# nem0/LumixEngine

Hardware: AMD Instinct MI355X
Metric: entities_culled_per_sec (higher is better)
Workload: dtype f32; 1 GPU; BASELINE config 2: 10000000 static entities per GPU (sparse, cube +-15000), 1 frustum (fov 60, 16:9, near 0.1, far 10000), cull + compaction; entities_per_gpu=10000000, frusta=1, repetitions=1

## Files before the change

lumixengine_amd/csrc/cull_kernels.hip:

```cpp
#include <algorithm>
#include <cstddef>
#include <cstdlib>

#include "lmx_kernels.h"
#include <type_traits>

#include <hip/hip_ext.h>

namespace lmx {

namespace {

__device__ __forceinline__ uint32_t lane_id() { return __builtin_amdgcn_mbcnt_hi(~0u, __builtin_amdgcn_mbcnt_lo(~0u, 0u)); }
__device__ __forceinline__ uint32_t mbcnt64(uint64_t mask) {
	return __builtin_amdgcn_mbcnt_hi((uint32_t)(mask >> 32), __builtin_amdgcn_mbcnt_lo((uint32_t)mask, 0u));
}
typedef uint32_t u32x4_a4 __attribute__((ext_vector_type(4), aligned(4)));
__device__ __forceinline__ float readlane_f(float v, int lane) { return __uint_as_float(__builtin_amdgcn_readlane(__float_as_uint(v), lane)); }

struct TileScalars {
	uint32_t ent_begin, cell_cap, n_frusta;
	uint32_t keys_packed;
	uint32_t out_stride, cnt_pad, cnt_frustum_stride, n_zero;
	int32_t* out_slots;
// ... 65 lines not shown
	const double cs = (double)CELL_SIZE;
	const double ox = org[0], oy = org[1], oz = org[2];
	const float lx = (float)(cs * bi[0] - cs - ox), ly = (float)(cs * bi[1] - cs - oy), lz = (float)(cs * bi[2] - cs - oz);
	const float hx = (float)(cs * bi[3] + cs - ox), hy = (float)(cs * bi[4] + cs - oy), hz = (float)(cs * bi[5] + cs - oz);
	const float clx = (float)(cs * bi[0] + cs - ox), cly = (float)(cs * bi[1] + cs - oy), clz = (float)(cs * bi[2] + cs - oz);
	const float chx = (float)(cs * bi[3] + 2 * cs - ox), chy = (float)(cs * bi[4] + 2 * cs - oy), chz = (float)(cs * bi[5] + 2 * cs - oz);
	const float b1 = max_f(abs_f(lx), abs_f(chx)) + max_f(abs_f(ly), abs_f(chy)) + max_f(abs_f(lz), abs_f(chz));
	const float n1 = abs_f(nx) + abs_f(ny) + abs_f(nz);
	const float margin = max_f(1.0f, n1) * (2.0f + 4e-6f * b1) + 1e-6f * abs_f(d);
	bool rej, in;
	{
		const float bx = nx > 0.0f ? hx : lx, by = ny > 0.0f ? hy : ly, bz = nz > 0.0f ? hz : lz;
		const float dp = (nx * bx) + (ny * by) + (nz * bz);
		rej = dp < -d - margin;
	}
	{
		const float bx = nx < 0.0f ? chx : clx, by = ny < 0.0f ? chy : cly, bz = nz < 0.0f ? chz : clz;
		const float dp = (nx * bx) + (ny * by) + (nz * bz);
		in = dp > -d + margin;
	}
	const uint64_t rej_mask = __ballot(plane_lane && rej), out_mask = __ballot(plane_lane && !in);
	uint32_t st_bits = 0;
	for (int g = 0; g < nf; ++g) {
		const uint32_t r = (uint32_t)(rej_mask >> (6 * g)) & 63u, o = (uint32_t)(out_mask >> (6 * g)) & 63u;
		st_bits |= (r != 0 ? (uint32_t)TILE_REJECT : (o == 0 ? (uint32_t)TILE_ACCEPT : (uint32_t)TILE_MIXED)) << (2 * g);
	}
	return st_bits;
}


typedef float v2f __attribute__((ext_vector_type(2)));
typedef float f32x16 __attribute__((ext_vector_type(16)));
typedef float v4f_t __attribute__((ext_vector_type(4)));
typedef uint32_t u32x4_t __attribute__((ext_vector_type(4)));
typedef __bf16 bf16x2_t __attribute__((ext_vector_type(2)));
typedef __bf16 bf16x8_t __attribute__((ext_vector_type(8)));
__device__ __forceinline__ uint32_t pk_bf16(float a, float b) { const v2f v = {a, b}; return __builtin_bit_cast(uint32_t, __builtin_convertvector(v, bf16x2_t)); }
typedef float v8f_t __attribute__((ext_vector_type(8)));
__device__ __forceinline__ float min3_drop_nan(float a, float b, float c) { return fminf(fminf(a, b), c); }
__device__ __forceinline__ bool sphere_visible_d_pk(const DevFrustum& f, const float d[6], float cx, float cy, float cz, float radius) {
	const v2f x2 = {cx, cx}, y2 = {cy, cy}, z2 = {cz, cz}, r2 = {radius, radius};
	bool culled = false;
#pragma unroll
	for (int k = 0; k < 6; k += 2) {
		const v2f nx = {f.nx[k], f.nx[k + 1]}, ny = {f.ny[k], f.ny[k + 1]}, nz = {f.nz[k], f.nz[k + 1]}, dd = {d[k], d[k + 1]};
		v2f t = x2 * nx;
		t = t + y2 * ny;
		t = t + z2 * nz;
		t = t + dd;
		t = t + r2;
		culled = culled || (t.x < 0) || (t.y < 0);
	}
	return !culled;
}


struct alignas(16) CellInfo { float d[6]; uint32_t cls, pad; };
static_assert(sizeof(CellInfo) == 32, "two ds_read_b128 per (lane, chunk, frustum)");

#ifndef LMX_ASM_SGPR
#define LMX_ASM_SGPR(x) "+s"(x)
#endif
#define LMX_CULL_WAVES_ATTR(F) __attribute__((amdgpu_waves_per_eu((F) == 1 ? 1 : 5)))

template <int F, int WAVES, int CHW, int GRP, int FORM, int SLOTS_I>
__global__ __launch_bounds__(WAVES * 64) LMX_CULL_WAVES_ATTR(F) void k_cull_tile(const FrustaArg fr_arg, const float4* __restrict__ g_spheres, const int32_t* __restrict__ g_ids,
	const ChunkHdr* __restrict__ g_hdr, const CellKey* __restrict__ g_tile_cells, const uint32_t* __restrict__ g_tile_tab, const TileBox* __restrict__ g_tile_box,
	const uint2* __restrict__ g_tile_out, int32_t* __restrict__ g_out_ids, uint32_t* __restrict__ g_counts, uint32_t* __restrict__ g_counts_next, const TileScalars a) {
	constexpr bool SLOTS = SLOTS_I != 0;
	constexpr uint32_t TILE = WAVES * CHW * 64;
	constexpr uint32_t THREADS = WAVES * 64;
	constexpr int FS = F == 1 ? 1 : MAX_FRUSTA;
	static_assert(CHW * FS <= 32, "visibility bits of a wave's chunks x frusta live in one register");
	LMX_DYNAMIC_LDS(CellInfo, s_info);
	__shared__ __attribute__((aligned(16))) float s_nrm[F != 1 ? MAX_FRUSTA : 1][F != 1 ? 20 : 4];
	const DevFrustum* __restrict__ frp = (const DevFrustum*)__builtin_amdgcn_kernarg_segment_ptr();
	const int nf = F == 1 ? 1 : (int)a.n_frusta;

	const uint32_t lane = lane_id();
	const uint32_t wave = __builtin_amdgcn_readfirstlane(threadIdx.x >> 6);
	const uint32_t tile_ent = a.ent_begin + blockIdx.x * TILE;
	const uint32_t tile_index = tile_ent / TILE;

	for (uint32_t i = blockIdx.x * THREADS + threadIdx.x; i < a.n_zero; i += gridDim.x * THREADS) g_counts_next[i] = 0;

	uint32_t st_bits = 0, tile_flags = 0, plane_skip = 0;
	bool any_mixed = false, any_live = false;
	if constexpr (FORM != 0) {
		static_assert(F == 1, "the lane-parallel tile test handles one frustum");
		__shared__ uint32_t s_verdict;
		if (wave == 0) {
			const uint32_t v = tile_status_lanes(g_tile_box + tile_index, lane);
			if (lane == 0) s_verdict = v;
		}
		__syncthreads();
		const uint32_t r = s_verdict;
		st_bits = r & 3u;
		tile_flags = (r >> 2) & 63u;
		plane_skip = __builtin_amdgcn_readfirstlane((r >> 8) & 63u);
		any_mixed = st_bits == TILE_MIXED;
		any_live = st_bits != TILE_REJECT;
	} else {
		__shared__ uint32_t s_verdict_multi[2];
		if (wave == 0) {
			uint32_t fl;
			const uint32_t v = tile_status_lanes_multi(g_tile_box + tile_index, lane, nf, &fl);
			if (lane == 0) {
				s_verdict_multi[0] = v;
				s_verdict_multi[1] = fl;
			}
		}
		__syncthreads();
		st_bits = __builtin_amdgcn_readfirstlane(s_verdict_multi[0]);
		tile_flags = __builtin_amdgcn_readfirstlane(s_verdict_multi[1]);
		static_assert(TILE_REJECT == 0 && TILE_ACCEPT == 1 && TILE_MIXED == 2, "the verdicts of all frusta are read off the 2-bit fields by bit logic");
		any_mixed = ((st_bits >> 1) & ~st_bits & 0x5555u) != 0;
		any_live = st_bits != 0;
	}
	if (!any_live) return;
	uint32_t tile_word = 0;
	v2f* s_d2 = reinterpret_cast<v2f*>(s_info);
	uint32_t* s_word = reinterpret_cast<uint32_t*>(s_d2 + (F != 1 ? (size_t)nf * a.cell_cap * 3 : 0));
	constexpr bool SPLIT = F != 1 && WAVES == 4;
	uint16_t* s_w16 = reinterpret_cast<uint16_t*>(s_word);
	if constexpr (F != 1) {
		static_assert(TILE_ACCEPT == 1 && CELL_ACCEPT == 1, "a settled frustum contributes CELL_ACCEPT or nothing: its verdict field IS its class field");
		tile_word = st_bits & ~(st_bits >> 1) & 0x5555u;
	}

	constexpr bool STREAMING = F == 1 && (FORM == 2 || FORM == 4);
	constexpr bool PRELOAD = STREAMING || F != 1;
	typedef float v4f_pre __attribute__((ext_vector_type(4)));
	v4f_pre pre_sp[PRELOAD ? GRP : 1];
	int32_t pre_id[PRELOAD ? GRP : 1];
	auto preload_group0 = [&](auto with_spheres) {
		if constexpr (PRELOAD) {
			const size_t e0 = ((size_t)((tile_ent >> 6) + wave * CHW) << 6) + lane;
#pragma unroll
			for (int i = 0; i < GRP; ++i) {
				pre_id[i] = __builtin_nontemporal_load(g_ids + e0 + i * 64);
				if constexpr (decltype(with_spheres)::value) pre_sp[i] = __builtin_nontemporal_load(reinterpret_cast<const v4f_pre*>(g_spheres + e0 + i * 64));
			}
		}
	};
	uint32_t first_cell = 0;
	if (any_mixed) {
		first_cell = g_tile_tab[2 * tile_index];
		const uint32_t n_cells = g_tile_tab[2 * tile_index + 1];
		const bool packed_keys = F == 1 ? FORM <= 2 : a.keys_packed != 0;
		const char* keys = reinterpret_cast<const char*>(g_tile_cells) + ((size_t)tile_index * a.cell_cap << (packed_keys ? 3 : 4));
		struct FetchedKey { uint4 raw; int32_t lo[3]; };
		auto fetch_key = [&](uint32_t t) -> FetchedKey {
			FetchedKey k;
			if (packed_keys) {
				const uint2 raw = reinterpret_cast<const uint2*>(keys)[t];
				k.raw = uint4{raw.x, raw.y, 0u, 0u};
				uint32_t zero = 0;
				asm volatile("" : "+v"(zero));
				const int32_t* box_lo = reinterpret_cast<const int32_t*>(g_tile_box + tile_index) + zero;
				k.lo[0] = box_lo[0]; k.lo[1] = box_lo[1]; k.lo[2] = box_lo[2];
			} else {
				k.raw = reinterpret_cast<const uint4*>(keys)[t];
				k.lo[0] = k.lo[1] = k.lo[2] = 0;
			}
			return k;
		};
		auto decode_key = [&](const FetchedKey& k) -> CellKey {
// ... 550 lines not shown

__global__ __launch_bounds__(256) void k_apply_patches(float4* __restrict__ spheres, int32_t* __restrict__ ids, TileBox* __restrict__ box0,
	TileBox* __restrict__ box1, TileBox* __restrict__ box2, DynDeviceView d, const PatchSphere* __restrict__ ps, uint32_t n_ps,
	const PatchId* __restrict__ pi, uint32_t n_pi, const PatchDyn* __restrict__ pd, uint32_t n_pd) {
	uint32_t i = blockIdx.x * 256u + threadIdx.x;
	if (i < n_ps) {
		const PatchSphere p = ps[i];
		spheres[p.slot] = make_float4(p.x, p.y, p.z, p.radius);
		return;
	}
	i -= n_ps;
	if (i < n_pi) {
		const PatchId p = pi[i];
		ids[p.slot] = p.id;
		if (p.id < 0) {
			atomicAnd(&box0[p.slot >> 12].flags, ~(uint32_t)TILE_DENSE);
			atomicAnd(&box1[p.slot >> 11].flags, ~(uint32_t)TILE_DENSE);
			atomicAnd(&box2[p.slot >> 10].flags, ~(uint32_t)TILE_DENSE);
		}
		return;
	}
	i -= n_pi;
	if (i < n_pd) {
		const PatchDyn p = pd[i];
		d.px[p.slot] = p.px;
		d.py[p.slot] = p.py;
		d.pz[p.slot] = p.pz;
		d.radius[p.slot] = p.radius;
		d.ids[p.slot] = p.id;
	}
}

constexpr int FIN_THREADS = 256;
constexpr int FIN_MAX_SHARDS = 1024;
__global__ __launch_bounds__(FIN_THREADS) void k_cull_finalize(const uint32_t* __restrict__ counts, uint32_t cnt_pad, uint32_t cnt_frustum_stride,
	const uint8_t* __restrict__ shard_type, uint32_t n_shards, uint32_t* __restrict__ totals, uint32_t* __restrict__ pref, uint32_t* __restrict__ packed_start) {
	__shared__ uint32_t s_cnt[FIN_MAX_SHARDS];
	__shared__ uint8_t s_type[FIN_MAX_SHARDS];
	__shared__ uint32_t s_tot[MAX_TYPES];
	const uint32_t f = blockIdx.x;
	const uint32_t t = threadIdx.x;
	if (t < MAX_TYPES) s_tot[t] = 0;
	for (uint32_t s = t; s < n_shards; s += FIN_THREADS) {
		s_cnt[s] = counts[f * cnt_frustum_stride + s * cnt_pad];
		s_type[s] = shard_type[s];
	}
	__syncthreads();
	for (uint32_t s = t; s < n_shards; s += FIN_THREADS) {
		const uint8_t ty = s_type[s];
		uint32_t run = 0;
		for (uint32_t k = s; k-- > 0 && s_type[k] == ty;) run += s_cnt[k];
		pref[f * n_shards + s] = run;
		if (s + 1 == n_shards || s_type[s + 1] != ty) s_tot[ty] = run + s_cnt[s];
	}
	__syncthreads();
	if (t < MAX_TYPES) {
		totals[f * MAX_TYPES + t] = s_tot[t];
		if (packed_start != nullptr) {
			uint32_t at = 0;
			for (uint32_t k = 0; k < t; ++k) at += s_tot[k];
			packed_start[f * MAX_TYPES + t] = at;
		}
	}
}

__global__ __launch_bounds__(256) void k_cull_consolidate(const int32_t* __restrict__ src, uint32_t src_stride, const uint32_t* __restrict__ win_base,
	const uint32_t* __restrict__ counts, uint32_t cnt_pad, uint32_t cnt_frustum_stride, const uint8_t* __restrict__ shard_type,
	const uint32_t* __restrict__ type_start, uint32_t type_start_stride, const uint32_t* __restrict__ pref, uint32_t n_shards, int32_t* __restrict__ dst,
	uint32_t dst_stride, uint32_t dst_cap, const int32_t* __restrict__ src2 ,
	int32_t* __restrict__ dst2) {
	const uint32_t s = blockIdx.x, f = blockIdx.y;
	const uint32_t c = counts[f * cnt_frustum_stride + s * cnt_pad];
	const size_t from_at = (size_t)f * src_stride + win_base[s];
	const uint32_t at = type_start[f * type_start_stride + shard_type[s]] + pref[f * n_shards + s];
	const size_t to_at = (size_t)f * dst_stride + at;
	const uint32_t room = at < dst_cap ? dst_cap - at : 0u;
	const uint32_t n = c < room ? c : room;
	for (uint32_t k = blockIdx.z * 256u + threadIdx.x; k < n; k += gridDim.z * 256u) {
		dst[to_at + k] = src[from_at + k];
		if (src2 != nullptr) dst2[to_at + k] = src2[from_at + k];
	}
}

__global__ __launch_bounds__(256) void k_cull_pack(const int32_t* __restrict__ src, const uint32_t* __restrict__ win_base, const uint32_t* __restrict__ counts,
	uint32_t cnt_pad, const uint8_t* __restrict__ shard_type, uint32_t n_shards, int32_t* __restrict__ rec_base, PackLayout lay,
	uint32_t src_stride, uint32_t cnt_stride) {
	__shared__ uint32_t s_part[4];
	__shared__ uint32_t s_tot[MAX_TYPES];
	const uint32_t s = blockIdx.x, t = threadIdx.x;
	src += (size_t)blockIdx.z * src_stride;
	counts += (size_t)blockIdx.z * cnt_stride;
	uint32_t* const header = reinterpret_cast<uint32_t*>(rec_base + lay.off[blockIdx.z]);
	int32_t* const dst = rec_base + lay.off[blockIdx.z] + MAX_TYPES;
	const uint32_t dst_cap = lay.cap[blockIdx.z];
	const bool totals_block = s == 0 && blockIdx.y == 0;
	const uint32_t c = counts[s * cnt_pad];
	if (blockIdx.y * 256u >= c && !totals_block) return;
	const int32_t* from = src + win_base[s];
	const uint32_t k0 = blockIdx.y * 256u + t;
	const int32_t first = k0 < c ? from[k0] : 0;
	uint32_t before = 0;
	for (uint32_t k = t; k < s; k += 256u) before += counts[k * cnt_pad];
#pragma unroll
	for (int o = 32; o > 0; o >>= 1) before += (uint32_t)__shfl_xor((int)before, o);
	if ((t & 63u) == 0) s_part[t >> 6] = before;
	if (totals_block && t < MAX_TYPES) s_tot[t] = 0;
	__syncthreads();
	const uint32_t at = s_part[0] + s_part[1] + s_part[2] + s_part[3];
	if (totals_block) {
		for (uint32_t k = t; k < n_shards; k += 256u) atomicAdd(&s_tot[shard_type[k]], counts[k * cnt_pad]);
		__syncthreads();
		if (t < MAX_TYPES) header[t] = s_tot[t];
	}
	int32_t* to = dst + at;
	const uint32_t room = at < dst_cap ? dst_cap - at : 0u;
	const uint32_t n = c < room ? c : room;
	if (k0 < n) to[k0] = first;
	for (uint32_t k = k0 + gridDim.y * 256u; k < n; k += gridDim.y * 256u) to[k] = from[k];
}

template <int F, int WAVES, int CHW, int GRP, int FORM, int SLOTS_I>
hipError_t tile_f(hipStream_t s, const CullDeviceView& v, uint32_t ent_begin, uint32_t ent_end, const TypeTable& tt, const FrustaArg& fr, int n_frusta,
	const CullOut& out) {
	constexpr uint32_t TILE = WAVES * CHW * 64;
	static_assert(TILE_ALIGN % TILE == 0, "tiles must not straddle type ranges");
	constexpr int K = TILE == 4096 ? 0 : (TILE == 2048 ? 1 : 2);
	const uint32_t tiles = (ent_end - ent_begin) / TILE;
	if (!tiles) {
		if (out.ev_start != nullptr) {
			(void)hipEventRecord(out.ev_start, s);
			(void)hipEventRecord(out.ev_stop, s);
		}
		return hipSuccess;
	}
	TileScalars a;
	(void)tt;
	a.ent_begin = ent_begin;
	a.cell_cap = v.tile_cap[K];
	a.keys_packed = v.keys_packed ? 1u : 0u;
	a.n_frusta = (uint32_t)n_frusta;
	a.out_stride = out.stride;
	a.cnt_pad = out.cnt_pad;
	a.cnt_frustum_stride = out.cnt_frustum_stride;
	a.n_zero = out.n_zero;
	a.out_slots = out.slots;
	{
		float n1 = 0.f;
		bool finite = true;
		for (int f = 0; f < n_frusta; ++f) {
			for (int k = 0; k < 6; ++k) {
				const float v = (__builtin_fabsf(fr.f[f].nx[k]) + __builtin_fabsf(fr.f[f].ny[k])) + __builtin_fabsf(fr.f[f].nz[k]);
				finite = finite && v <= 3.0e38f;
				n1 = v > n1 ? v : n1;
			}
		}
		a.pretest_n1s = finite ? n1 * 1.000001f * 134217728.0f : __builtin_inff();
	}
	if (out.ev_start != nullptr)
		hipExtLaunchKernelGGL((k_cull_tile<F, WAVES, CHW, GRP, FORM, SLOTS_I>), dim3(tiles), dim3(WAVES * 64), cull_tile_lds_bytes(n_frusta, a.cell_cap), s, out.ev_start, out.ev_stop, 0, fr,
			v.spheres, v.ids, v.hdr, v.tile_cells[K], v.tile_tab[K], v.tile_box[K], v.tile_out[K], out.ids, out.counts, out.counts_next, a);
	else
		hipLaunchKernelGGL((k_cull_tile<F, WAVES, CHW, GRP, FORM, SLOTS_I>), dim3(tiles), dim3(WAVES * 64), cull_tile_lds_bytes(n_frusta, a.cell_cap), s, fr, v.spheres, v.ids, v.hdr,
			v.tile_cells[K], v.tile_tab[K], v.tile_box[K], v.tile_out[K], out.ids, out.counts, out.counts_next, a);
	return hipGetLastError();
}

}

size_t cull_tile_lds_bytes(int n_frusta, uint32_t cell_cap) {
	return n_frusta > 1 ? (size_t)n_frusta * cell_cap * 24 + (size_t)cell_cap * (n_frusta > 4 ? 8 : 4) : (size_t)cell_cap * sizeof(CellInfo);
}

uint32_t cull_tile_size(int n_frusta, int variant) {
	(void)variant;
	return n_frusta <= 4 ? 2048u : 1024u;
}

hipError_t launch_cull_tile(hipStream_t s, const CullDeviceView& v, uint32_t ent_begin, uint32_t ent_end, const TypeTable& tt, const FrustaArg& fr,
	int n_frusta, const CullOut& out, int variant) {
#define LMX_TILE(F, W, C, G, L) return out.slots ? tile_f<F, W, C, G, L, 1>(s, v, ent_begin, ent_end, tt, fr, n_frusta, out) : tile_f<F, W, C, G, L, 0>(s, v, ent_begin, ent_end, tt, fr, n_frusta, out)
	if (n_frusta < 1 || n_frusta > MAX_FRUSTA) return hipErrorInvalidValue;
	if (n_frusta == 1) {
		const int wide = v.keys_packed ? 0 : 2;
		if (variant == 4) { if (wide) LMX_TILE(1, 4, 8, 8, 3); LMX_TILE(1, 4, 8, 8, 1); }
		if (wide) LMX_TILE(1, 4, 8, 4, 4);
		LMX_TILE(1, 4, 8, 4, 2);
	}
	if (n_frusta <= 4) LMX_TILE(0, 8, 4, 4, 0);
	LMX_TILE(0, 4, 4, 4, 0);
#undef LMX_TILE
}

uint32_t cull_dynamic_tile(int n_frusta, uint32_t n_slots) {
	uint32_t tile = n_frusta <= 2 ? 2048u : (n_frusta <= 4 ? 1024u : 512u);
	while (tile > 256u && n_slots / tile < 2048u) tile >>= 1;
	return tile;
}

__global__ __launch_bounds__(256) void k_dyn_carry_over(const double* __restrict__ opx, const double* __restrict__ opy, const double* __restrict__ opz,
	const float* __restrict__ oradius, const int32_t* __restrict__ oids, uint32_t n_old, double* __restrict__ npx, double* __restrict__ npy, double* __restrict__ npz,
	float* __restrict__ nradius, const int32_t* __restrict__ nids, uint32_t n_new, const int32_t* __restrict__ new_slot_of_entity, uint32_t n_entities) {
	const uint32_t s = blockIdx.x * 256u + threadIdx.x;
	if (s >= n_old) return;
	const int32_t e = oids[s];
	if (e < 0 || (uint32_t)e >= n_entities) return;
	const int32_t t = new_slot_of_entity[e];
	if (t < 0 || (uint32_t)t >= n_new || nids[t] != e) return;
	npx[t] = opx[s];
	npy[t] = opy[s];
	npz[t] = opz[s];
	nradius[t] = oradius[s];
}

hipError_t launch_dyn_carry_over(hipStream_t s, const DynDeviceView& from, const DynDeviceView& to, const int32_t* new_slot_of_entity, uint32_t n_entities) {
	if (!from.n_padded || !to.n_padded || !n_entities) return hipSuccess;
	hipLaunchKernelGGL(k_dyn_carry_over, dim3((from.n_padded + 255u) / 256u), dim3(256), 0, s, from.px, from.py, from.pz, from.radius, from.ids, from.n_padded, to.px, to.py,
		to.pz, to.radius, to.ids, to.n_padded, new_slot_of_entity, n_entities);
	return hipGetLastError();
}

hipError_t launch_cull_dynamic(hipStream_t s, const DynDeviceView& d, uint32_t slot_begin, uint32_t slot_end, const TypeTable& dyn_tt,
	const FrustaArg& fr, int n_frusta, const CullOut& out) {
	const uint32_t tile = cull_dynamic_tile(n_frusta, slot_end - slot_begin);
	const uint32_t blocks = (slot_end - slot_begin) / tile;
	if (!blocks) return hipSuccess;
	const size_t lds = (size_t)n_frusta * tile * sizeof(int32_t) + 2 * MAX_FRUSTA * sizeof(uint32_t);
#define LMX_DYN(T) hipLaunchKernelGGL(k_cull_dynamic<T>, dim3(blocks), dim3(DYN_THREADS), lds, s, d.px, d.py, d.pz, d.radius, d.ids, fr, n_frusta, dyn_tt, slot_begin, out)
	if (tile == 2048) LMX_DYN(2048);
	else if (tile == 1024) LMX_DYN(1024);
	else if (tile == 512) LMX_DYN(512);
	else LMX_DYN(256);
#undef LMX_DYN
	return hipGetLastError();
}

hipError_t launch_apply_patches(hipStream_t s, float4* spheres, int32_t* ids, TileBox* const tile_box[3], const DynDeviceView& d, const PatchSphere* ps,
	uint32_t n_ps, const PatchId* pi, uint32_t n_pi, const PatchDyn* pd, uint32_t n_pd) {
	const uint32_t n = n_ps + n_pi + n_pd;
	if (!n) return hipSuccess;
	hipLaunchKernelGGL(k_apply_patches, dim3((n + 255u) / 256u), dim3(256), 0, s, spheres, ids, tile_box[0], tile_box[1], tile_box[2], d, ps, n_ps, pi, n_pi, pd, n_pd);
	return hipGetLastError();
}

hipError_t launch_cull_finalize(hipStream_t s, const uint32_t* counts, uint32_t cnt_pad, uint32_t cnt_frustum_stride, const uint8_t* shard_type,
	uint32_t n_shards, uint32_t n_frusta, uint32_t* totals, uint32_t* pref, uint32_t* packed_start) {
	if (!n_frusta) return hipSuccess;
	if (n_shards > (uint32_t)FIN_MAX_SHARDS) return hipErrorInvalidValue;
	hipLaunchKernelGGL(k_cull_finalize, dim3(n_frusta), dim3(FIN_THREADS), 0, s, counts, cnt_pad, cnt_frustum_stride, shard_type, n_shards, totals, pref, packed_start);
	return hipGetLastError();
}

hipError_t launch_cull_consolidate(hipStream_t s, const int32_t* src, uint32_t src_stride, const uint32_t* win_base, const uint32_t* counts,
	uint32_t cnt_pad, uint32_t cnt_frustum_stride, const uint8_t* shard_type, const uint32_t* type_start, uint32_t type_start_stride, const uint32_t* pref,
	uint32_t n_shards, uint32_t n_frusta, uint32_t max_shard_cap, int32_t* dst, uint32_t dst_stride, uint32_t dst_cap, const int32_t* src2, int32_t* dst2) {
	if (!n_frusta || !n_shards) return hipSuccess;
	const uint32_t splits = std::max(1u, std::min(64u, max_shard_cap / 4096u));
	hipLaunchKernelGGL(k_cull_consolidate, dim3(n_shards, n_frusta, splits), dim3(256), 0, s, src, src_stride, win_base, counts, cnt_pad, cnt_frustum_stride,
		shard_type, type_start, type_start_stride, pref, n_shards, dst, dst_stride, dst_cap, src2, dst2);
	return hipGetLastError();
}

hipError_t launch_cull_pack_layout(hipStream_t s, const int32_t* src, const uint32_t* win_base, const uint32_t* counts, uint32_t cnt_pad, const uint8_t* shard_type,
	uint32_t n_shards, uint32_t max_shard_cap, int32_t* rec_base, const PackLayout& lay, uint32_t n_frusta, uint32_t src_stride, uint32_t cnt_stride) {
	if (!n_frusta) return hipSuccess;
	if (n_frusta > (uint32_t)MAX_FRUSTA) return hipErrorInvalidValue;
	if (!n_shards) {
		for (uint32_t f = 0; f < n_frusta; ++f)
			if (hipError_t e = hipMemsetAsync(rec_base + lay.off[f], 0, MAX_TYPES * sizeof(uint32_t), s)) return e;
		return hipSuccess;
	}
	if (n_shards > (uint32_t)FIN_MAX_SHARDS) return hipErrorInvalidValue;
	const uint32_t splits = std::max(1u, std::min(64u, max_shard_cap / 4096u));
	hipLaunchKernelGGL(k_cull_pack, dim3(n_shards, splits, n_frusta), dim3(256), 0, s, src, win_base, counts, cnt_pad, shard_type, n_shards, rec_base, lay, src_stride,
		cnt_stride);
	return hipGetLastError();
}

hipError_t launch_cull_pack(hipStream_t s, const int32_t* src, const uint32_t* win_base, const uint32_t* counts, uint32_t cnt_pad, const uint8_t* shard_type,
	uint32_t n_shards, uint32_t max_shard_cap, uint32_t* header, int32_t* dst, uint32_t dst_cap, uint32_t n_frusta, uint32_t src_stride, uint32_t cnt_stride,
	uint32_t rec_stride) {
	if (n_frusta > (uint32_t)MAX_FRUSTA || dst != reinterpret_cast<int32_t*>(header) + MAX_TYPES) return hipErrorInvalidValue;
	PackLayout lay = {};
	for (uint32_t f = 0; f < n_frusta; ++f) {
		lay.off[f] = (uint64_t)f * rec_stride;
		lay.cap[f] = dst_cap;
	}
	return launch_cull_pack_layout(s, src, win_base, counts, cnt_pad, shard_type, n_shards, max_shard_cap, reinterpret_cast<int32_t*>(header), lay, n_frusta, src_stride, cnt_stride);
}

}
```

lumixengine_amd/csrc/lmx_capi_cull.hip:

```cpp
#include "lmx_cull_host.h"

#include <optional>

using namespace lmx;

namespace {

static_assert(sizeof(LayoutSphere) == sizeof(float4) && sizeof(LayoutCell) == sizeof(CellKey) && sizeof(LayoutChunkHdr) == sizeof(ChunkHdr), "layout PODs mirror the device types");
static_assert(LAYOUT_MAX_TYPES == MAX_TYPES && LAYOUT_CHUNK == CHUNK && LAYOUT_TILE_ALIGN == TILE_ALIGN && LAYOUT_CELL_DEAD == CELL_DEAD, "layout constants");

constexpr uint32_t DYN_ALIGN = 2048;
constexpr uint32_t DYN_MAX_SHARDS = 8;

CullDeviceView static_view(const CullSet& cs) {
	CullDeviceView v;
	v.spheres = cs.spheres.p;
	v.ids = cs.ids.p;
	v.hdr = cs.hdr.p;
	v.n_padded = cs.n_padded;
	v.keys_packed = cs.keys_packed;
	for (int k = 0; k < 3; ++k) {
		v.tile_cells[k] = cs.tile_cells[k].p;
		v.tile_tab[k] = cs.tile_tab[k].p;
		v.tile_box[k] = cs.tile_box[k].p;
// ... 376 lines not shown
	});
	return cull_flush(ctx);
}

int lmx_cull_flush(LmxContext* ctx) {
	LMX_CHECK_CTX(ctx);
	return cull_flush(ctx);
}

int lmx_cull_compact(LmxContext* ctx) {
	LMX_CHECK_CTX(ctx);
	return flush_impl(ctx, true);
}

int lmx_cull_stats(LmxContext* ctx, uint32_t* n_entities, uint32_t* n_cells, uint32_t* n_chunks) {
	LMX_CHECK_CTX(ctx);
	if (int rc = flush_impl(ctx, true)) return rc;
	const CullState& cs = ctx->cull;
	if (n_entities) *n_entities = (uint32_t)(cs.recs.size() + cs.dyn.size());
	if (n_cells) *n_cells = cs.n_cells - cs.n_dead_cells;
	if (n_chunks) *n_chunks = (cs.out_total + CHUNK - 1) / CHUNK;
	return LMX_OK;
}

int lmx_cull_layout_info(LmxContext* ctx, uint32_t* cell_key_bytes, uint64_t* table_bytes) {
	LMX_CHECK_CTX(ctx);
	if (int rc = flush_impl(ctx, true)) return rc;
	const CullState& cs = ctx->cull;
	const uint32_t kb = cs.keys_packed ? (uint32_t)sizeof(PackedCellKey) : (uint32_t)sizeof(CellKey);
	if (cell_key_bytes) *cell_key_bytes = kb;
	if (table_bytes) {
		const uint64_t tiles = cs.n_padded / 2048u;
		*table_bytes = tiles * ((uint64_t)cs.tile_cap[1] * kb + 2 * sizeof(uint32_t) + sizeof(TileBox) + sizeof(uint2)) + (uint64_t)(cs.n_padded / CHUNK) * sizeof(ChunkHdr);
	}
	return LMX_OK;
}

int lmx_cull_update_stats(LmxContext* ctx, uint32_t* n_static, uint32_t* n_dynamic_bound, uint32_t* n_overflow, uint32_t* n_tombstones) {
	LMX_CHECK_CTX(ctx);
	const CullState& cs = ctx->cull;
	if (n_static) *n_static = (uint32_t)cs.recs.size();
	if (n_dynamic_bound) *n_dynamic_bound = (uint32_t)(cs.dyn.size() - cs.n_unbound);
	if (n_overflow) *n_overflow = cs.n_unbound;
	if (n_tombstones) *n_tombstones = cs.n_tombstones;
	return LMX_OK;
}

static double frustum_box_overlap(const CullState& cs, const LmxShiftedFrustum& f) {
	if (cs.big_tile_fraction > 0.5) return 1.0;
	double vol_scene = 1, vol_overlap = 1;
	for (int a = 0; a < 3; ++a) {
		double lo = INFINITY, hi = -INFINITY;
		for (int k = 0; k < 8; ++k) {
			const double p = f.origin[a] + (double)f.points[k][a];
			lo = std::min(lo, p);
			hi = std::max(hi, p);
		}
		const double extent = cs.scene_hi[a] - cs.scene_lo[a];
		if (!(extent > 0) || !(hi >= lo)) return 1.0;
		vol_scene *= extent;
		vol_overlap *= std::max(0.0, std::min(hi, cs.scene_hi[a]) - std::max(lo, cs.scene_lo[a]));
	}
	return vol_overlap / vol_scene;
}

int lmx_cull(LmxContext* ctx, uint32_t view, const LmxShiftedFrustum* frusta, uint32_t n_frusta, uint8_t type) {
	LMX_CHECK_CTX(ctx);
	if (view >= LMX_MAX_VIEWS) return fail(ctx, LMX_ERR_CAPACITY, "view %u >= LMX_MAX_VIEWS", view);
	if (!frusta || n_frusta == 0 || n_frusta > LMX_MAX_FRUSTA) return fail(ctx, LMX_ERR_CAPACITY, "n_frusta %u not in [1,%d]", n_frusta, LMX_MAX_FRUSTA);
	if (type != LMX_TYPE_ALL && type >= MAX_TYPES) return fail(ctx, LMX_ERR_CAPACITY, "type %u >= LMX_MAX_TYPES", type);
	if (int rc = cull_flush(ctx)) return rc;
	CullState& cs = ctx->cull;
	CullView& v = cs.views[view];
	if (v.ext_out && v.ext_out_cap < (size_t)cs.out_total * n_frusta)
		return fail(ctx, LMX_ERR_CAPACITY, "bound output holds %zu ids, need %zu", v.ext_out_cap, (size_t)cs.out_total * n_frusta);
	const uint32_t cnt_frustum_stride = cs.n_shards * cs.cnt_pad;
	const uint32_t cnt_words = std::max(1u, MAX_FRUSTA * cnt_frustum_stride);
	if (v.cnt_words != cnt_words) {
		LMX_HIP(ctx, v.counts.reserve(2 * (size_t)cnt_words));
		v.cnt_words = cnt_words;
		v.flip = 0;
		LMX_HIP(ctx, hipMemsetAsync(v.counts.p, 0, 2 * (size_t)cnt_words * sizeof(uint32_t), ctx->stream));
		v.next_half_is_zero = true;
	}
	LMX_HIP(ctx, v.out.reserve(std::max<size_t>((size_t)cs.out_total * n_frusta, 1)));
	if (cs.emit_slots) LMX_HIP(ctx, v.out_slots.reserve(std::max<size_t>((size_t)cs.out_total * n_frusta, 1)));
	v.has_slots = cs.emit_slots;
	v.n_frusta = n_frusta;
	v.out_stride = cs.out_total;
	v.valid = v.finalized = v.consolidated = false;
	for (int t = 0; t < MAX_TYPES; ++t) {
		v.out_start[t] = cs.type_start[t];
		v.out_cap[t] = cs.type_cap[t];
	}
	FrustaArg fr;
	memset(&fr, 0, sizeof(fr));
	for (uint32_t f = 0; f < n_frusta; ++f) fr.f[f] = to_dev_frustum(frusta[f]);

	uint32_t ent_begin = 0, ent_end = cs.n_padded, dyn_begin = 0, dyn_end = cs.dyn_padded;
	if (type != LMX_TYPE_ALL) {
		ent_begin = cs.tt.ent_start[type];
		ent_end = cs.tt.ent_end[type];
		dyn_begin = cs.dyn_tt.ent_start[type];
		dyn_end = cs.dyn_tt.ent_end[type];
	}
	v.flip ^= 1u;
	if (!v.next_half_is_zero) LMX_HIP(ctx, hipMemsetAsync(v.counts_ptr(), 0, (size_t)cnt_words * sizeof(uint32_t), ctx->stream));
	v.next_half_is_zero = ent_end > ent_begin;
	CullOut out;
	out.ids = v.out.p;
	out.stride = v.out_stride;
	out.win_base = cs.d_win_base.p;
	out.counts = v.counts_ptr();
	out.cnt_pad = cs.cnt_pad;
	out.cnt_frustum_stride = cnt_frustum_stride;
	out.counts_next = v.counts_other();
	out.n_zero = cnt_words;
	out.slots = cs.emit_slots ? v.out_slots.p : nullptr;
	CullDeviceView dv = static_view(cs);
	for (int k = 0; k < 3; ++k) dv.tile_out[k] = cs.d_tile_out[k].p;
	const uint32_t pass_width = cs.pass_width ? cs.pass_width : (ent_end - ent_begin <= (1u << 25) ? n_frusta : 1u);
	for (uint32_t f0 = 0; f0 < n_frusta; f0 += pass_width) {
		const uint32_t fw = std::min(pass_width, n_frusta - f0);
		FrustaArg sub;
		memset(&sub, 0, sizeof(sub));
		for (uint32_t k = 0; k < fw; ++k) sub.f[k] = fr.f[f0 + k];
		CullOut po = out;
		po.ids = out.ids + (size_t)f0 * out.stride;
		if (out.slots) po.slots = out.slots + (size_t)f0 * out.stride;
		po.counts = out.counts + (size_t)f0 * cnt_frustum_stride;
		if (f0 != 0) {
			po.counts_next = nullptr;
			po.n_zero = 0;
		}
		const int variant = cs.tile_variant >= 0 ? cs.tile_variant : (fw == 1 && frustum_box_overlap(cs, frusta[f0]) < 0.25 ? 4 : 1);
		ProfScope ps(ctx, LMX_K_CULL_SPHERES, true);
		po.ev_start = ps.slot.a;
		po.ev_stop = ps.slot.b;
		const hipError_t launched = launch_cull_tile(ctx->stream, dv, ent_begin, ent_end, cs.tt, sub, (int)fw, po, variant);
		if (launched != hipSuccess) ps.cancel();
		LMX_HIP(ctx, launched);
	}
	if (dyn_end > dyn_begin) {
		CullOut po = out;
		po.counts_next = nullptr;
		po.n_zero = 0;
		ProfScope ps(ctx, LMX_K_CULL_DYNAMIC);
		LMX_HIP(ctx, launch_cull_dynamic(ctx->stream, dyn_view(cs), dyn_begin, dyn_end, cs.dyn_tt, fr, (int)n_frusta, po));
	}
	v.valid = true;
	if (v.ext_out) return cull_view_consolidate(ctx, v);
	return LMX_OK;
}

int lmx_cull_set_pass_width(LmxContext* ctx, uint32_t frusta_per_pass) {
	LMX_CHECK_CTX(ctx);
	if (frusta_per_pass > LMX_MAX_FRUSTA) return fail(ctx, LMX_ERR_INVALID_ARGUMENT, "pass width %u not in [0,%d]", frusta_per_pass, LMX_MAX_FRUSTA);
	ctx->cull.pass_width = frusta_per_pass;
	return LMX_OK;
}

int lmx_cull_set_option(LmxContext* ctx, int option, int value) {
	LMX_CHECK_CTX(ctx);
	CullState& cs = ctx->cull;
	switch (option) {
		case LMX_CULL_OPT_TILE_VARIANT:
			if (value != -1 && value != 1 && value != 4) return fail(ctx, LMX_ERR_INVALID_ARGUMENT, "tile variant %d: -1 (auto), 1 (streaming) or 4 (all loads in flight)", value);
			cs.tile_variant = value;
			return LMX_OK;
		case LMX_CULL_OPT_AUTO_COMPACTION: cs.auto_compaction = value != 0; return LMX_OK;
		case LMX_CULL_OPT_COMPACTION_MIN:
			if (value < 1) return fail(ctx, LMX_ERR_INVALID_ARGUMENT, "compaction minimum %d < 1", value);
			cs.compaction_min = (uint32_t)value;
			return LMX_OK;
		case LMX_CULL_OPT_DEVICE_OWNS_BOUND: cs.device_owns_bound = value != 0; return LMX_OK;
		case LMX_CULL_OPT_MAP_ZERO_COPY: cs.map_zero_copy = value != 0; cs.map_zero_copy_max = value > 1 ? (uint32_t)value : (1u << 20); return LMX_OK;
		case LMX_CULL_OPT_ASYNC_COMPACTION:
			if (value) return async_enable(ctx);
			async_disable(cs);
			return LMX_OK;
		case LMX_CULL_OPT_OVERFLOW_RESERVE:
			if (value < 0) return fail(ctx, LMX_ERR_INVALID_ARGUMENT, "overflow reserve %d < 0", value);
			cs.overflow_reserve = (uint32_t)value;
			if (value) {
				cs.dyn_layout_dirty = true;
				const size_t ids = std::max(cs.ent_to_dyn.size(), cs.ent_to_rec.size());
				cs.ent_to_dyn.reserve(ids + (size_t)value);
				if (cs.ent_to_dyn.size() < ids) cs.ent_to_dyn.resize(ids, -1);
				cs.dyn.reserve(cs.dyn.size() + (size_t)value);
			}
			return LMX_OK;
		case LMX_CULL_OPT_MAX_SHARDS:
			if (value < 1 || value > (int)LAYOUT_MAX_SHARDS) return fail(ctx, LMX_ERR_INVALID_ARGUMENT, "max shards %d not in [1,%u]", value, LAYOUT_MAX_SHARDS);
			cs.max_shards = (uint32_t)value;
			if (cs.built) return recompute_out_layout(ctx);
			return LMX_OK;
		case LMX_CULL_OPT_COUNTER_PAD:
			if (value < 1 || value > 64) return fail(ctx, LMX_ERR_INVALID_ARGUMENT, "counter pad %d not in [1,64]", value);
			cs.cnt_pad = (uint32_t)value;
			for (CullView& v : cs.views) {
// ... 10 lines not shown
```

lumixengine_amd/csrc/lmx_context.h:

```cpp
#pragma once

#include <hip/hip_runtime.h>

#include <algorithm>
#include <cstdarg>
#include <cstdio>
#include <cstdlib>
#include <cstring>
#include <atomic>
#include <condition_variable>
#include <mutex>
#include <string>
#include <unordered_map>
#include <vector>

#include "lumix_mi355.h"
#include "lmx_kernels.h"
#include "lmx_cull_layout.h"

namespace lmx {

template <typename T> struct DevBuf {
	T* p = nullptr;
	size_t cap = 0;
	~DevBuf() { release(); }
	void release() {
		if (p) (void)hipFree(p);
		p = nullptr;
		cap = 0;
	}
	DevBuf() = default;
	DevBuf(const DevBuf&) = delete;
	DevBuf& operator=(const DevBuf&) = delete;
	DevBuf(DevBuf&& o) noexcept { swap(o); }
	DevBuf& operator=(DevBuf&& o) noexcept {
		if (this != &o) {
			release();
			swap(o);
		}
		return *this;
	}
	void swap(DevBuf& o) {
		std::swap(p, o.p);
		std::swap(cap, o.cap);
	}
	hipError_t reserve(size_t n) {
		if (n <= cap) return hipSuccess;
		release();
		const size_t want = n + n / 8 + 64;
		hipError_t e = hipMalloc((void**)&p, want * sizeof(T));
		if (e != hipSuccess) {
			p = nullptr;
			return e;
		}
		cap = want;
		return hipSuccess;
	}
};


template <typename T> hipError_t upload_blocking(T* dst, const T* src, size_t n) { return n ? hipMemcpy(dst, src, n * sizeof(T), hipMemcpyHostToDevice) : hipSuccess; }
template <typename T> hipError_t upload_blocking(DevBuf<T>& dst, const T* src, size_t n) {
	const hipError_t e = dst.reserve(std::max<size_t>(n, 1));
	return e != hipSuccess ? e : upload_blocking(dst.p, src, n);
}
template <typename D, typename T> hipError_t upload_blocking(D&& dst, const std::vector<T>& src) { return upload_blocking(dst, src.data(), src.size()); }

template <typename T> hipError_t upload_on_stream(T* dst, const T* src, size_t n, hipStream_t stream) { return n ? hipMemcpyAsync(dst, src, n * sizeof(T), hipMemcpyHostToDevice, stream) : hipSuccess; }
template <typename T> hipError_t upload_on_stream(DevBuf<T>& dst, const T* src, size_t n, hipStream_t stream) {
	const hipError_t e = dst.reserve(std::max<size_t>(n, 1));
	return e != hipSuccess ? e : upload_on_stream(dst.p, src, n, stream);
}
template <typename D, typename T> hipError_t upload_on_stream(D&& dst, const std::vector<T>& src, hipStream_t stream) { return upload_on_stream(dst, src.data(), src.size(), stream); }

template <typename T> hipError_t read_back(T* dst, const T* src, size_t n, hipStream_t stream) { return n && dst ? hipMemcpyAsync(dst, src, n * sizeof(T), hipMemcpyDeviceToHost, stream) : hipSuccess; }

template <typename T> hipError_t device_copy_blocking(T* dst, const T* src, size_t n) { return n ? hipMemcpy(dst, src, n * sizeof(T), hipMemcpyDeviceToDevice) : hipSuccess; }
template <typename T> hipError_t device_copy_on_stream(T* dst, const T* src, size_t n, hipStream_t stream) { return n ? hipMemcpyAsync(dst, src, n * sizeof(T), hipMemcpyDeviceToDevice, stream) : hipSuccess; }

struct CullView {
	DevBuf<int32_t> out;
	DevBuf<uint32_t> counts;
	DevBuf<uint32_t> totals;
	DevBuf<uint32_t> pref;
	DevBuf<int32_t> cons;
	DevBuf<int32_t> out_slots, cons_slots;
	bool has_slots = false;
	uint32_t n_frusta = 0;
	uint32_t out_stride = 0;
	uint32_t cnt_words = 0;
	uint32_t out_start[MAX_TYPES] = {};
	uint32_t out_cap[MAX_TYPES] = {};
	bool valid = false;
	bool finalized = false;
	bool consolidated = false;
	int32_t* ext_out = nullptr;
	size_t ext_out_cap = 0;
	uint32_t* ext_counts = nullptr;
	uint32_t flip = 0;
	bool next_half_is_zero = false;
	void* map_host = nullptr;
	size_t map_words = 0;
	std::atomic<uint32_t> map_guess[LMX_MAX_FRUSTA] = {{4096}, {4096}, {4096}, {4096}, {4096}, {4096}, {4096}, {4096}};
	bool map_seen = false;
	size_t map_frusta = 0;
	DevBuf<int32_t> map_rec;
	hipEvent_t map_event = nullptr;
	struct MapTicket {
		uint32_t first = 0, n = 0;
		bool zero_copy = false;
		int32_t* host = nullptr;
		const int32_t* rec = nullptr;
		size_t words = 0;
		size_t guess[LMX_MAX_FRUSTA] = {};
		uint32_t out_cap[MAX_TYPES] = {};
	} ticket;
	DevBuf<uint32_t> map_pref, map_start;
	DevBuf<int32_t> pack_rec;
	size_t pack_words = 0;
	~CullView() {
		if (map_host) (void)hipHostFree(map_host);
		if (map_event) (void)hipEventDestroy(map_event);
	}
	CullView() = default;
	CullView(const CullView&) = delete;
	CullView& operator=(const CullView&) = delete;
	uint32_t* counts_ptr() const { return counts.p + flip * cnt_words; }
	uint32_t* counts_other() const { return counts.p + (flip ^ 1u) * cnt_words; }
	const int32_t* cons_ptr() const { return ext_out ? ext_out : cons.p; }
	const uint32_t* totals_ptr() const { return ext_counts ? ext_counts : totals.p; }
};

struct DynRec {
	double pos[3];
	float radius;
	int32_t entity;
	uint32_t slot;
	uint8_t type;
	bool bound;
};
constexpr uint32_t DYN_NO_SLOT = 0xffffffffu;

struct PatchStaging {
	void* host[2] = {nullptr, nullptr};
	void* dev[2] = {nullptr, nullptr};
	size_t cap[2] = {0, 0};
	hipEvent_t done[2] = {nullptr, nullptr};
	uint32_t next = 0;
	PatchStaging() = default;
	PatchStaging(const PatchStaging&) = delete;
	PatchStaging& operator=(const PatchStaging&) = delete;
	PatchStaging(PatchStaging&& o) noexcept { swap(o); }
	PatchStaging& operator=(PatchStaging&& o) noexcept {
		swap(o);
		return *this;
	}
	void swap(PatchStaging& o) {
		for (int i = 0; i < 2; ++i) {
			std::swap(host[i], o.host[i]);
			std::swap(dev[i], o.dev[i]);
			std::swap(cap[i], o.cap[i]);
			std::swap(done[i], o.done[i]);
		}
		std::swap(next, o.next);
	}
	~PatchStaging() {
		for (int i = 0; i < 2; ++i) {
			if (host[i]) (void)hipHostFree(host[i]);
			if (done[i]) (void)hipEventDestroy(done[i]);
		}
	}
};

struct CullSet {
	std::vector<CullRec> recs;
	std::vector<int32_t> ent_to_rec;
	std::vector<uint32_t> rec_slot;
	bool structure_dirty = false;
	bool built = false;
	uint32_t n_tombstones = 0;
	DevBuf<float4> spheres;
	DevBuf<int32_t> ids;
	DevBuf<ChunkHdr> hdr;
// ... 367 lines not shown
```

Measured before the change: 678.4 billion entities/s.

## Vectorize pack copy, use wave-level prefix sums, and zero only used count rows

The pack kernel now computes each shard's output offset and the per-type totals with wave-level DPP reductions instead of LDS, shared atomics and block barriers. It copies with 16-byte vector loads and stores, unrolled four deep, and sizes the split count toward a fixed total number of blocks. The cull kernel now zeroes only the padded count slots that the previous frame actually used, tracked per half, instead of the full count buffer. The goal is to cut pack-kernel latency and redundant zeroing stores. The price is more complex bookkeeping and unaligned vector accesses.

```diff
diff --git a/lumixengine_amd/csrc/cull_kernels.hip b/lumixengine_amd/csrc/cull_kernels.hip
--- a/lumixengine_amd/csrc/cull_kernels.hip
+++ b/lumixengine_amd/csrc/cull_kernels.hip
@@ -171,7 +171,7 @@
 	const uint32_t tile_ent = a.ent_begin + blockIdx.x * TILE;
 	const uint32_t tile_index = tile_ent / TILE;
 
-	for (uint32_t i = blockIdx.x * THREADS + threadIdx.x; i < a.n_zero; i += gridDim.x * THREADS) g_counts_next[i] = 0;
+	for (uint32_t i = blockIdx.x * THREADS + threadIdx.x; i < a.n_zero; i += gridDim.x * THREADS) g_counts_next[i * a.cnt_pad] = 0;
 
 	uint32_t st_bits = 0, tile_flags = 0, plane_skip = 0;
 	bool any_mixed = false, any_live = false;
@@ -888,41 +888,89 @@
 	}
 }
 
+constexpr uint32_t PACK_SPAN = 256u * 4u;
+constexpr uint32_t PACK_BLOCKS = 1024u;
+__device__ __forceinline__ uint32_t wave_sum(uint32_t v) {
+	v += (uint32_t)__builtin_amdgcn_mov_dpp((int)v, 0xB1, 0xf, 0xf, true);
+	v += (uint32_t)__builtin_amdgcn_mov_dpp((int)v, 0x4E, 0xf, 0xf, true);
+	v += (uint32_t)__builtin_amdgcn_mov_dpp((int)v, 0x141, 0xf, 0xf, true);
+	v += (uint32_t)__builtin_amdgcn_mov_dpp((int)v, 0x140, 0xf, 0xf, true);
+	return (uint32_t)__builtin_amdgcn_readlane((int)v, 0) + (uint32_t)__builtin_amdgcn_readlane((int)v, 16) + (uint32_t)__builtin_amdgcn_readlane((int)v, 32) +
+		(uint32_t)__builtin_amdgcn_readlane((int)v, 48);
+}
 __global__ __launch_bounds__(256) void k_cull_pack(const int32_t* __restrict__ src, const uint32_t* __restrict__ win_base, const uint32_t* __restrict__ counts,
 	uint32_t cnt_pad, const uint8_t* __restrict__ shard_type, uint32_t n_shards, int32_t* __restrict__ rec_base, PackLayout lay,
 	uint32_t src_stride, uint32_t cnt_stride) {
-	__shared__ uint32_t s_part[4];
-	__shared__ uint32_t s_tot[MAX_TYPES];
-	const uint32_t s = blockIdx.x, t = threadIdx.x;
+	const uint32_t s = blockIdx.x, t = threadIdx.x, lane = t & 63u;
 	src += (size_t)blockIdx.z * src_stride;
 	counts += (size_t)blockIdx.z * cnt_stride;
-	uint32_t* const header = reinterpret_cast<uint32_t*>(rec_base + lay.off[blockIdx.z]);
-	int32_t* const dst = rec_base + lay.off[blockIdx.z] + MAX_TYPES;
+	const uint32_t win = win_base[s];
+	const uint64_t rec_off = lay.off[blockIdx.z];
 	const uint32_t dst_cap = lay.cap[blockIdx.z];
-	const bool totals_block = s == 0 && blockIdx.y == 0;
-	const uint32_t c = counts[s * cnt_pad];
-	if (blockIdx.y * 256u >= c && !totals_block) return;
-	const int32_t* from = src + win_base[s];
-	const uint32_t k0 = blockIdx.y * 256u + t;
-	const int32_t first = k0 < c ? from[k0] : 0;
-	uint32_t before = 0;
-	for (uint32_t k = t; k < s; k += 256u) before += counts[k * cnt_pad];
-#pragma unroll
-	for (int o = 32; o > 0; o >>= 1) before += (uint32_t)__shfl_xor((int)before, o);
-	if ((t & 63u) == 0) s_part[t >> 6] = before;
-	if (totals_block && t < MAX_TYPES) s_tot[t] = 0;
-	__syncthreads();
-	const uint32_t at = s_part[0] + s_part[1] + s_part[2] + s_part[3];
-	if (totals_block) {
-		for (uint32_t k = t; k < n_shards; k += 256u) atomicAdd(&s_tot[shard_type[k]], counts[k * cnt_pad]);
-		__syncthreads();
-		if (t < MAX_TYPES) header[t] = s_tot[t];
-	}
-	int32_t* to = dst + at;
+	const bool totals_wave = s == 0 && blockIdx.y == 0 && t < 64u;
+	uint32_t sum = 0, own = 0;
+	for (uint32_t b = 0; b <= s && !totals_wave; b += 256u) {
+		uint32_t v[4];
+#pragma unroll
+		for (uint32_t j = 0; j < 4; ++j) v[j] = b + 64u * j + lane <= s ? counts[(b + 64u * j + lane) * cnt_pad] : 0u;
+#pragma unroll
+		for (uint32_t j = 0; j < 4; ++j) {
+			sum += v[j];
+			own = b + 64u * j + lane == s ? v[j] : own;
+		}
+	}
+	if (totals_wave) {
+		uint32_t tot[MAX_TYPES] = {};
+		for (uint32_t b = 0; b < n_shards; b += 256u) {
+			uint32_t v[4], ty[4];
+#pragma unroll
+			for (uint32_t j = 0; j < 4; ++j) {
+				const bool in = b + 64u * j + lane < n_shards;
+				v[j] = in ? counts[(b + 64u * j + lane) * cnt_pad] : 0u;
+				ty[j] = in ? shard_type[b + 64u * j + lane] : 0u;
+			}
+			if (b == 0 && lane == 0) sum = own = v[0];
+#pragma unroll
+			for (uint32_t j = 0; j < 4; ++j)
+#pragma unroll
+				for (uint32_t y = 0; y < (uint32_t)MAX_TYPES; ++y) tot[y] += ty[j] == y ? v[j] : 0u;
+		}
+		uint32_t mine = 0;
+#pragma unroll
+		for (uint32_t y = 0; y < (uint32_t)MAX_TYPES; ++y) {
+			const uint32_t all = wave_sum(tot[y]);
+			mine = lane == y ? all : mine;
+		}
+		if (lane < (uint32_t)MAX_TYPES) reinterpret_cast<uint32_t*>(rec_base + rec_off)[lane] = mine;
+	}
+	const uint32_t c = (uint32_t)__builtin_amdgcn_readlane((int)own, s & 63u);
+	const uint32_t at = wave_sum(sum) - c;
 	const uint32_t room = at < dst_cap ? dst_cap - at : 0u;
 	const uint32_t n = c < room ? c : room;
-	if (k0 < n) to[k0] = first;
-	for (uint32_t k = k0 + gridDim.y * 256u; k < n; k += gridDim.y * 256u) to[k] = from[k];
+	const int32_t* const from = src + win;
+	int32_t* const to = rec_base + rec_off + MAX_TYPES + at;
+	const uint32_t step = gridDim.y * PACK_SPAN;
+	uint32_t b = blockIdx.y * PACK_SPAN;
+	for (; b + 3u * step + PACK_SPAN <= n; b += 4u * step) {
+		u32x4_a4 v[4];
+#pragma unroll
+		for (uint32_t j = 0; j < 4; ++j) v[j] = *reinterpret_cast<const u32x4_a4*>(from + (b + j * step + t * 4u));
+#pragma unroll
+		for (uint32_t j = 0; j < 4; ++j) *reinterpret_cast<u32x4_a4*>(to + (b + j * step + t * 4u)) = v[j];
+	}
+	for (; b < n; b += step) {
+		const uint32_t k = b + t * 4u;
+		if (k + 4u <= n) *reinterpret_cast<u32x4_a4*>(to + k) = *reinterpret_cast<const u32x4_a4*>(from + k);
+		else {
+			int32_t r[3];
+#pragma unroll
+			for (uint32_t i = 0; i < 3; ++i)
+				if (k + i < n) r[i] = from[k + i];
+#pragma unroll
+			for (uint32_t i = 0; i < 3; ++i)
+				if (k + i < n) to[k + i] = r[i];
+		}
+	}
 }
 
 template <int F, int WAVES, int CHW, int GRP, int FORM, int SLOTS_I>
@@ -1076,7 +1124,8 @@
 		return hipSuccess;
 	}
 	if (n_shards > (uint32_t)FIN_MAX_SHARDS) return hipErrorInvalidValue;
-	const uint32_t splits = std::max(1u, std::min(64u, max_shard_cap / 4096u));
+	const uint32_t want = (PACK_BLOCKS + n_shards * n_frusta - 1u) / (n_shards * n_frusta), spans = (max_shard_cap + PACK_SPAN - 1u) / PACK_SPAN;
+	const uint32_t splits = std::max(1u, std::min(want, spans));
 	hipLaunchKernelGGL(k_cull_pack, dim3(n_shards, splits, n_frusta), dim3(256), 0, s, src, win_base, counts, cnt_pad, shard_type, n_shards, rec_base, lay, src_stride,
 		cnt_stride);
 	return hipGetLastError();
diff --git a/lumixengine_amd/csrc/lmx_capi_cull.hip b/lumixengine_amd/csrc/lmx_capi_cull.hip
--- a/lumixengine_amd/csrc/lmx_capi_cull.hip
+++ b/lumixengine_amd/csrc/lmx_capi_cull.hip
@@ -482,6 +482,7 @@
 		v.flip = 0;
 		LMX_HIP(ctx, hipMemsetAsync(v.counts.p, 0, 2 * (size_t)cnt_words * sizeof(uint32_t), ctx->stream));
 		v.next_half_is_zero = true;
+		v.half_rows[0] = v.half_rows[1] = 0;
 	}
 	LMX_HIP(ctx, v.out.reserve(std::max<size_t>((size_t)cs.out_total * n_frusta, 1)));
 	if (cs.emit_slots) LMX_HIP(ctx, v.out_slots.reserve(std::max<size_t>((size_t)cs.out_total * n_frusta, 1)));
@@ -507,6 +508,7 @@
 	v.flip ^= 1u;
 	if (!v.next_half_is_zero) LMX_HIP(ctx, hipMemsetAsync(v.counts_ptr(), 0, (size_t)cnt_words * sizeof(uint32_t), ctx->stream));
 	v.next_half_is_zero = ent_end > ent_begin;
+	v.half_rows[v.flip] = n_frusta;
 	CullOut out;
 	out.ids = v.out.p;
 	out.stride = v.out_stride;
@@ -515,7 +517,8 @@
 	out.cnt_pad = cs.cnt_pad;
 	out.cnt_frustum_stride = cnt_frustum_stride;
 	out.counts_next = v.counts_other();
-	out.n_zero = cnt_words;
+	out.n_zero = v.half_rows[v.flip ^ 1u] * cs.n_shards;
+	if (v.next_half_is_zero) v.half_rows[v.flip ^ 1u] = 0;
 	out.slots = cs.emit_slots ? v.out_slots.p : nullptr;
 	CullDeviceView dv = static_view(cs);
 	for (int k = 0; k < 3; ++k) dv.tile_out[k] = cs.d_tile_out[k].p;
diff --git a/lumixengine_amd/csrc/lmx_context.h b/lumixengine_amd/csrc/lmx_context.h
--- a/lumixengine_amd/csrc/lmx_context.h
+++ b/lumixengine_amd/csrc/lmx_context.h
@@ -99,6 +99,7 @@
 	uint32_t* ext_counts = nullptr;
 	uint32_t flip = 0;
 	bool next_half_is_zero = false;
+	uint32_t half_rows[2] = {};
 	void* map_host = nullptr;
 	size_t map_words = 0;
 	std::atomic<uint32_t> map_guess[LMX_MAX_FRUSTA] = {{4096}, {4096}, {4096}, {4096}, {4096}, {4096}, {4096}, {4096}};
```

Measured after the change: 798.4 billion entities/s (median of 3 runs). +17.7%, better.
